# wittyseok/multimodal-organ-segmentation

Hardware: AMD Instinct MI355X
Metric: 96^3 2-modality patches/sec/node (train step) (higher is better)
Workload: dtype bf16; 1 GPU; DualEncoder fusion=cross_attention (mean, dual_encoder.py:193-195) 96^3, modalities CT+PET, 6 classes, DiceCE, AdamW, per-GPU batch 2; model=dual_encoder, global_batch=2, parallelism=dp1, kernels=hip, tag=c3

## Files before the change

include/mmseg_hip.h:

```cpp
#ifndef MMSEG_HIP_H
#define MMSEG_HIP_H

#include <stddef.h>
#include <stdint.h>

#ifdef __cplusplus
extern "C" {
#endif

const char* mmseg_last_error(void);
const char* mmseg_last_kernel(void);
int mmseg_abi_version(void);
int mmseg_timing_begin(void);
int mmseg_timing_end(void);
long long mmseg_timing_count(void);
int mmseg_timing_get(long long i, float* ms, const char** name);


int mmseg_pack_weight(const float* w, void* dst, int mode, int Co, int Ci, int Cip, int KG, int KGp, int Cpad,
                      int dtype, void* stream);

int mmseg_pack3_desc_bytes(void);
int mmseg_pack_conv3_batched(const void* descs, int n, int nblocks, int dtype, void* stream);
int mmseg_pack_desc_bytes(void);
// ... 58 lines not shown
                        const float* wdq, const float* bias, void* out, int ldo, int M, int Ncols, int Cpad, int KG,
                        int cpg_shift, int D, int H, int W, void* stream);
int mmseg_conv3_wgrad_norm_ok(long long V, int Co, int Cip, int Ci, int cpg_shift, int D, int H, int W, int lddy,
                              int ldx, int dtype);
int mmseg_conv3_wgrad_norm(const void* dy, int lddy, const void* x, int ldx, const float* nmean, const float* nrstd,
                           float* grad, float* bias_grad, int Co, int Cip, int Ci, int cpg_shift, long long V, int D,
                           int H, int W, float* ws, long long ws_floats, int accumulate, int dtype, void* stream);
int mmseg_conv_gemm_group(const void* a, int lda, const void* wpacked, const float* bias, void* out, int ldo,
                          float* splitk_ws, int mode, int M, int Ncols, int Cpad, int KG, int cpg_shift, int D, int H,
                          int W, int ksplit, int cin_real, int groups, long long w_gstride, int b_gstride, int dtype,
                          void* stream);
int mmseg_conv3_group_ok(int M, int Ncols, int Cpad, int KG, int cpg_shift, int D, int H, int W, int lda, int ldo,
                         int dtype);
int mmseg_conv3_wgrad_group_ok(long long V, int Co, int Cip, int Ci, int cpg_shift, int D, int H, int W, int lddy,
                               int ldx, int dtype);
int mmseg_conv3_group_splits(int M, int Ncols, int Cpad, int KG, int cpg_shift, int D, int H, int W, int lda, int ldo,
                             int dtype);
long long mmseg_conv3_wgrad_group_ws_floats(long long V, int Co, int Cip, int Ci, int cpg_shift, int D, int H, int W,
                                            int lddy, int ldx, int groups, int dtype);
int mmseg_conv3_wgrad_group(const void* dy, int lddy, const void* x, int ldx, float* grad, float* bias_grad, int Co,
                            int Cip, int Ci, int cpg_shift, long long V, int D, int H, int W, float* ws,
                            long long ws_floats, int accumulate, int groups, long long grad_gstride,
                            int bias_gstride, int phase, int dtype, void* stream);
int mmseg_wgrad_reduce_flush(void* stream);
int mmseg_wgrad_reduce_defer(const float* part, float* grad, const float* bias_part, float* bias_grad, int Ca,
                             int Ncols, int ksplit, int cpad, int creal, int ntap, int accumulate, void* stream);
int mmseg_wgrad_reduce_pending(void);
int mmseg_wgrad_reduce_discard(void* stream);
int mmseg_conv3_wgrad_ex(const void* dy, int lddy, const void* x, int ldx, const float* nmean, const float* nrstd,
                         float* grad, float* bias_grad, int Co, int Cip, int Ci, int cpg_shift, long long V, int D,
                         int H, int W, float* ws, long long ws_floats, int accumulate, int phase, int dtype,
                         void* stream);
int mmseg_colsum(const void* dy, int ld, int C, long long V, float* part, int nblk, float* out, int accumulate,
                 int dtype, void* stream);
int mmseg_colsum_reduce(const float* part, int nblk, int C, float* out, int accumulate, void* stream);

long long mmseg_instnorm_ws_floats(int N, long long V, int C);
int mmseg_instnorm_stats(const void* x, int ldx, int N, long long V, int C, float eps, float* mean, int mean_ld,
                         float* rstd, float* ws, int dtype, void* stream);
int mmseg_instnorm_relu_fwd(const void* x, int ldx, void* y, int ldy, int N, long long V, int C, const float* mean,
                            const float* rstd, int dtype, void* stream);
int mmseg_instnorm_relu_bwd_group(const void* x, int ldx, const float* mean, const float* rstd, const void* p1,
                                  int ld1, float scale1, int p1_nmod, const void* pool_dy, int pool_ld,
                                  const uint8_t* pool_idx, void* dx, int lddx, int N, int D, int H, int W, int C,
                                  float* ws, int dtype, void* stream);
int mmseg_instnorm_relu_bwd(const void* x, int ldx, const float* mean, const float* rstd, const void* p1, int ld1,
                            float scale1, const float* alpha1, int alpha_stride, const float* beta, int beta_stride,
                            const void* pool_dy, int pool_ld, const uint8_t* pool_idx, void* dx, int lddx, int N,
                            int D, int H, int W, int C, float* ws, int dtype, void* stream);
int mmseg_instnorm_act_bwd(const void* x, int ldx, const float* mean, const float* rstd, const void* g, int ldg,
                           void* dx, int lddx, int N, int D, int H, int W, int C, int Cw, int act, float slope,
                           const float* part, int nchunk, float* ws, int dtype, void* stream);
int mmseg_instnorm_part_chunks(long long V, int C);
int mmseg_lrelu_bwd_in_part(const void* y, int ldy, const void* dy, int lddy, void* g, int ldg, float slope,
                            const void* xa, int lda, const float* ma, const float* ra, float* pa, const void* xb,
                            int ldb, const float* mb, const float* rb, float* pb, int N, long long V, int C, int Cw,
                            int dtype, void* stream);
int mmseg_instnorm_fwd(const void* x, int ldx, void* y, int ldy, int N, long long V, int C, float eps, float* mean,
                       int mean_ld, float* rstd, int relu, float* ws, int dtype, void* stream);
int mmseg_instnorm_apply(const void* x, int ldx, void* y, int ldy, int N, long long V, int C, const float* mean,
                         const float* rstd, int relu, int dtype, void* stream);
int mmseg_instnorm_bwd(const void* x, int ldx, const float* mean, const float* rstd, const void* p1, int ld1,
                       float scale1, const float* alpha1, int alpha_stride, const float* beta, int beta_stride,
                       const void* pool_dy, int pool_ld, const uint8_t* pool_idx, void* dx, int lddx, int N, int D,
                       int H, int W, int C, int relu, float* ws, int dtype, void* stream);
int mmseg_instnorm_bwd_part(const void* x, int ldx, const float* mean, const float* rstd, const void* p1, int ld1,
                            float scale1, const float* alpha1, int alpha_stride, const float* beta, int beta_stride,
                            const void* pool_dy, int pool_ld, const uint8_t* pool_idx, void* dx, int lddx, int N,
                            int D, int H, int W, int C, int relu, const float* part, int nchunk, float* ws,
                            int dtype, void* stream);
int mmseg_instnorm_bwd_coef(const void* x, int ldx, const float* mean, const float* rstd, const void* p1, int ld1,
                            int N, int D, int H, int W, int C, int relu, const float* part, int nchunk,
                            float* coef, float* ws, int dtype, void* stream);
int mmseg_maxpool2_fwd(const void* x, int ldx, void* y, int ldy, uint8_t* idx, int N, int D, int H, int W, int C,
                       int dtype, void* stream);
int mmseg_maxpool2_norm_fwd(const void* x, int ldx, const float* mean, const float* rstd, void* y, int ldy,
                            uint8_t* idx, int N, int D, int H, int W, int C, int dtype, void* stream);

int mmseg_fuse_fwd(const void* const* srcs, const int* lds, int M, float wconst, const float* wts, void* out, int ldo,
                   int N, long long V, int C, int dtype, void* stream);
int mmseg_fuse_norm_fwd(const void* const* srcs, const int* lds, const float* const* means, const float* const* rstds,
                        int M, float wconst, const float* wts, void* out, int ldo, int N, long long V, int C,
                        int dtype, void* stream);
int mmseg_attn_gate_fwd(const float* pooled, const float* W1, const float* b1, const float* W2, const float* b2,
                        float* hbuf, float* wts, int N, int MC, int Hd, int M, void* stream);
int mmseg_attn_gate_bwd(const void* const* srcs, const int* lds, int M, const void* dfused, int ldd, int N, long long V,
                        int C, const float* pooled, const float* W1, const float* W2, const float* hbuf,
                        const float* wts, float* beta, float* gW1, float* gb1, float* gW2, float* gb2, int Hd,
                        float* ws, int accumulate, int dtype, void* stream);

int mmseg_bgemm_nt(const void* a, long long sa_outer, long long sa_inner, int lda, const void* b, long long sb_outer,
                   long long sb_inner, int ldb, void* c, long long sc_outer, long long sc_inner, int ldc,
                   const float* bias, int batch, int inner, int M, int N, int K, float alpha, int accumulate,
                   int c_dtype, int dtype, void* stream);
int mmseg_transpose(const void* src, long long s_outer, long long s_inner, int lds, int src_dtype, void* dst,
                    long long d_outer, long long d_inner, int ldd, int dst_dtype, int batch, int inner, int rows,
                    int cols, void* stream);
int mmseg_softmax_rows(const float* S, int lds, void* P, int ldp, long long rows, int N, int dtype, void* stream);
int mmseg_softmax_bwd_rows(const void* P, int ldp, const float* dP, int lddp, void* dS, int ldds, long long rows,
                           int N, int dtype, void* stream);

int mmseg_relpos_bias(const float* table, const int* index, int heads, int N, float* bias, void* stream);
int mmseg_softmax_bias_rows(const float* S, int lds, const float* bias, const float* mask, int nw, int heads, void* P,
                            int ldp, long long rows, int N, int dtype, void* stream);
int mmseg_relpos_table_grad(const void* dS, int ldn, int B, int heads, int N, float* dB, const int* offs,
                            const int* pairs, int T, float* gtable, int accumulate, int dtype, void* stream);

long long mmseg_winattn_lse_floats(int B, int heads);
int mmseg_winattn_fwd(const void* qkv, int B, int N, int C, int heads, const float* table, int T, int w0, int w1,
                      int w2, const uint8_t* region, int nw, float scale, void* O, float* lse, void* stream);
int mmseg_winattn_bwd(const void* qkv, const void* O, const void* dO, const float* lse, int B, int N, int C, int heads,
                      const float* table, int T, int w0, int w1, int w2, const uint8_t* region, int nw, float scale,
                      void* dqkv, void* dS, int ldn, void* stream);
int mmseg_winattn_sum_groups(int B, int N, int heads);
int mmseg_winattn_bwd_sum(const void* qkv, const void* O, const void* dO, const float* lse, int B, int N, int C,
                          int heads, const float* table, int T, int w0, int w1, int w2, const uint8_t* region, int nw,
                          float scale, void* dqkv, float* dsum, int ldn, void* stream);

int mmseg_layernorm_fwd(const void* x, int ldx, void* y, int ldy, long long rows, int C, const float* gamma,
                        const float* beta, float eps, float* mean, float* rstd, int dtype, void* stream);
long long mmseg_layernorm_bwd_ws_floats(long long rows, int C);
int mmseg_layernorm_bwd(const void* x, int ldx, const void* dy, int lddy, void* dx, int lddx, long long rows, int C,
                        const float* gamma, const float* mean, const float* rstd, int add_dx, float* dgamma,
                        float* dbeta, int accumulate, float* ws, int dtype, void* stream);
int mmseg_gelu_fwd(const void* h, void* y, long long n, int dtype, void* stream);
int mmseg_gelu_bwd(const void* h, const void* dy, void* dh, long long n, int dtype, void* stream);
int mmseg_add(const void* a, const void* b, void* out, long long n, int dtype, void* stream);
int mmseg_dropout(const void* x, void* y, long long rows, int C, long long V, int ncdhw, float p, long long seed,
                  int dtype, void* stream);
int mmseg_window_partition(const void* src, int ldx, int B, int D, int H, int W, int C, int w0, int w1, int w2,
                           int s0, int s1, int s2, int Dp, int Hp, int Wp, void* dst, int dtype, void* stream);
int mmseg_window_reverse(const void* win, int B, int D, int H, int W, int C, int w0, int w1, int w2, int s0, int s1,
                         int s2, int Dp, int Hp, int Wp, const void* add_src, int ld_add, void* dst, int ld_dst,
                         int dtype, void* stream);
int mmseg_merge_gather(const void* x, int ldx, int B, int D, int H, int W, int C, void* out, int dtype, void* stream);
int mmseg_merge_scatter(const void* dout, int B, int D, int H, int W, int C, void* dx, int lddx, int dtype,
                        void* stream);
int mmseg_patchify(const float* x, int B, int Cin, int D, int H, int W, int Kp, void* out, int dtype, void* stream);
int mmseg_res_apply(const void* a, int lda, const float* ma, const float* ra, const void* b, int ldb, const float* mb,
                    const float* rb, void* y, int ldy, int N, long long V, int C, int Cw, float slope, int dtype,
                    void* stream);
int mmseg_lrelu_bwd(const void* y, int ldy, const void* dy, int lddy, void* g, int ldg, long long rows, int C, int Cw,
                    float slope, int dtype, void* stream);

long long mmseg_normalize_ws_bytes(void);
int mmseg_modality_normalize(float* x, long long V, int kind, double lo, double hi, void* ws, void* stream);
int mmseg_resize_linear(const float* src, int C, int D, int H, int W, float* dst, int d, int h, int w, void* stream);
int mmseg_resize_nearest(const void* src, int label_bytes, int C, int D, int H, int W, void* dst, int d, int h, int w,
                         void* stream);
int mmseg_phantom(int S, int ncls, const double* geo, int M, const float* class_mean, const float* noise_sd,
                  const int* abs_noise, const unsigned long long* keys, void* label, int label_bytes, float* image,
                  void* stream);
int mmseg_augment(const float* src, int C, int D, int H, int W, const void* label, int label_bytes, int flip_mask,
                  int rot_k, const float* scale, const float* shift, int noise, double noise_mean, float noise_sd,
                  const unsigned long long* noise_key, float* dst, void* label_dst, void* stream);

int mmseg_window_gather(const float* vol, int N, int C, int D, int H, int W, const int* win, int nw, int r0, int r1,
                        int r2, float* out, void* stream);
int mmseg_window_accum(const float* logits, int N, int C, int D, int H, int W, int n, int z0, int y0, int x0, int r0,
                       int r1, int r2, float* out, void* stream);
int mmseg_window_norm(float* out, int N, int C, int D, int H, int W, const float* cz, const float* cy, const float* cx,
                      void* stream);

int mmseg_pack_input(const float* x, int Ctot, int c0, int cnt, int N, long long V, void* out, int dtype,
                     void* stream);
int mmseg_pack_input_compact(const float* x, int Ctot, int c0, int cnt, int N, long long V, void* out, int dtype,
// ... 70 lines not shown
```

multimodal-organ-segmentation_amd/csrc/norm_pool.hip:

```cpp
#include "mmseg_common.h"

#include <algorithm>

#include <stdlib.h>
#include <type_traits>

namespace {

constexpr int UNR = 4;

template <typename T>
__global__ void in_stats_partial(const T* __restrict__ x, int ld, int V, int C, int vpc, float* __restrict__ part) {
  const int n = blockIdx.y, chunk = blockIdx.x, nchunk = gridDim.x;
  const int C8 = C >> 3;
  const int lanes_v = 256 / C8;
  const int tid = threadIdx.x;
  const int cg = tid % C8, vl = tid / C8;
  const T* xn = x + (long long)n * V * ld + cg * 8;
  float mu[8], m2[8];
#pragma unroll
  for (int j = 0; j < 8; ++j) {
    mu[j] = 0.f;
    m2[j] = 0.f;
  }
// ... 1026 lines not shown
  int M;
  float wconst;
  const float* wts;
  const float* mean[4];
  const float* rstd[4];
};

template <typename T, bool NORM = false>
__global__ void fuse_fwd(FuseSrc s, T* __restrict__ out, int ldo, long long V, int N, int C) {
  const int C8 = C >> 3;
  const int total = N * (int)V * C8;
  for (int i = blockIdx.x * blockDim.x + threadIdx.x; i < total; i += gridDim.x * blockDim.x) {
    const int cg = i % C8;
    const long long nv = i / C8;
    const int n = (int)(nv / (int)V);
    float acc[8];
#pragma unroll
    for (int j = 0; j < 8; ++j) acc[j] = 0.f;
    for (int m = 0; m < s.M; ++m) {
      V8<T> a;
      a.load(reinterpret_cast<const T*>(s.p[m]) + nv * s.ld[m] + cg * 8);
      if constexpr (NORM) {
        float mu[8], rs[8];
        load8f(s.mean[m] + n * C + cg * 8, mu);
        load8f(s.rstd[m] + n * C + cg * 8, rs);
#pragma unroll
        for (int j = 0; j < 8; ++j) {
          const float h = (a.get(j) - mu[j]) * rs[j];
          a.set(j, h > 0.f ? h : 0.f);
        }
      }
      const float w = s.wts ? s.wts[n * s.M + m] : 1.f;
#pragma unroll
      for (int j = 0; j < 8; ++j) acc[j] = s.wts ? fmaf(a.get(j), w, acc[j]) : acc[j] + a.get(j);
    }
    V8<T> o;
#pragma unroll
    for (int j = 0; j < 8; ++j) o.set(j, s.wts ? acc[j] : acc[j] * s.wconst);
    o.store(out + nv * ldo + cg * 8);
  }
}

template <typename T, int MM>
__global__ void fuse_norm_fwd_m(FuseSrc s, T* __restrict__ out, int ldo, long long V, int N, int C) {
  const int C8 = C >> 3;
  const int total = N * (int)V * C8;
  const int stride = gridDim.x * blockDim.x;
  int i = blockIdx.x * blockDim.x + threadIdx.x;
  const int cg = i % C8;
  int cur_n = -1;
  float mu[MM][8], rs[MM][8];
  for (; i < total; i += stride) {
    const long long nv = i / C8;
    const int n = (int)(nv / (int)V);
    V8<T> a[MM];
#pragma unroll
    for (int m = 0; m < MM; ++m) a[m].load(reinterpret_cast<const T*>(s.p[m]) + nv * s.ld[m] + cg * 8);
    if (n != cur_n) {
#pragma unroll
      for (int m = 0; m < MM; ++m) {
        load8f(s.mean[m] + n * C + cg * 8, mu[m]);
        load8f(s.rstd[m] + n * C + cg * 8, rs[m]);
      }
      cur_n = n;
    }
    float acc[8];
#pragma unroll
    for (int j = 0; j < 8; ++j) acc[j] = 0.f;
#pragma unroll
    for (int m = 0; m < MM; ++m) {
#pragma unroll
      for (int j = 0; j < 8; ++j) {
        const float h = (a[m].get(j) - mu[m][j]) * rs[m][j];
        a[m].set(j, h > 0.f ? h : 0.f);
      }
      const float w = s.wts ? s.wts[n * s.M + m] : 1.f;
#pragma unroll
      for (int j = 0; j < 8; ++j) acc[j] = s.wts ? fmaf(a[m].get(j), w, acc[j]) : acc[j] + a[m].get(j);
    }
    V8<T> o;
#pragma unroll
    for (int j = 0; j < 8; ++j) o.set(j, s.wts ? acc[j] : acc[j] * s.wconst);
    o.store(out + nv * ldo + cg * 8);
  }
}

template <typename T>
__global__ void fuse_dot_partial(FuseSrc s, const T* __restrict__ dfused, int ldd, long long V, int C, long long vpc,
                                 float* __restrict__ part) {
  const int n = blockIdx.y, chunk = blockIdx.x, nchunk = gridDim.x;
  const int C8 = C >> 3;
  const int tid = threadIdx.x;
  float acc[4] = {0.f, 0.f, 0.f, 0.f};
  const long long v0 = (long long)chunk * vpc;
  long long v1 = v0 + vpc;
  if (v1 > V) v1 = V;
  const long long e0 = v0 * C8, e1 = v1 * C8;
  for (long long e = e0 + tid; e < e1; e += 256) {
    const long long v = e / C8;
    const int cg = (int)(e - v * C8);
    const long long nv = (long long)n * V + v;
    V8<T> d;
    d.load(dfused + nv * ldd + cg * 8);
    for (int m = 0; m < s.M; ++m) {
      V8<T> a;
      a.load(reinterpret_cast<const T*>(s.p[m]) + nv * s.ld[m] + cg * 8);
      float t = 0.f;
#pragma unroll
      for (int j = 0; j < 8; ++j) t = fmaf(a.get(j), d.get(j), t);
      acc[m] += t;
    }
  }
  __shared__ float red[4][4];
  const int lane = tid & 63, wave = tid >> 6;
  for (int m = 0; m < s.M; ++m) {
    float w = wave_sum(acc[m]);
    if (lane == 0) red[m][wave] = w;
  }
  __syncthreads();
  if (tid < s.M) part[((long long)n * nchunk + chunk) * 4 + tid] = red[tid][0] + red[tid][1] + red[tid][2] + red[tid][3];
}

__global__ void attn_gate_fwd(const float* __restrict__ pooled, const float* __restrict__ W1,
                              const float* __restrict__ b1, const float* __restrict__ W2, const float* __restrict__ b2,
                              float* __restrict__ hbuf, float* __restrict__ wts, int MC, int Hd, int M) {
  const int n = blockIdx.x;
  extern __shared__ float sh[];
  float* h = sh;
  for (int k = threadIdx.x; k < Hd; k += blockDim.x) {
    float a = 0.f;
    for (int i = 0; i < MC; ++i) a = fmaf(W1[(long long)k * MC + i], pooled[(long long)n * MC + i], a);
    a += b1[k];
    a = a > 0.f ? a : 0.f;
    h[k] = a;
    hbuf[(long long)n * Hd + k] = a;
  }
  __syncthreads();
  if (threadIdx.x == 0) {
    float lg[4];
    float mx = -INFINITY;
    for (int m = 0; m < M; ++m) {
      float a = 0.f;
      for (int k = 0; k < Hd; ++k) a = fmaf(W2[m * Hd + k], h[k], a);
      lg[m] = a + b2[m];
      mx = fmaxf(mx, lg[m]);
    }
    float se = 0.f;
    for (int m = 0; m < M; ++m) {
      lg[m] = expf(lg[m] - mx);
      se += lg[m];
    }
    for (int m = 0; m < M; ++m) wts[n * M + m] = lg[m] / se;
  }
}

__global__ void attn_gate_bwd(const float* __restrict__ dot_part, int nchunk, const float* __restrict__ pooled,
                              const float* __restrict__ W1, const float* __restrict__ W2,
                              const float* __restrict__ hbuf, const float* __restrict__ wts, float* __restrict__ beta,
                              float* __restrict__ gW1, float* __restrict__ gb1, float* __restrict__ gW2,
                              float* __restrict__ gb2, int N, int MC, int Hd, int M, long long V, int accumulate) {
  extern __shared__ float sh[];
  float* dlog = sh;
  float* dh = sh + N * M;
  const int tid = threadIdx.x;
  if (tid < N * M) {
    const int n = tid / M, m = tid % M;
// ... 399 lines not shown
int mmseg_maxpool2_fwd(const void* x, int ldx, void* y, int ldy, uint8_t* idx, int N, int D, int H, int W, int C,
                       int dtype, void* stream) {
  MMSEG_REQUIRE(C % 8 == 0 && ((D | H | W) & 1) == 0, "maxpool2: C%%8==0 and even dims required");
  MMSEG_REQUIRE((long long)N * (D / 2) * (H / 2) * (W / 2) * (C / 8) <= kGridStrideMax, "maxpool2: too many items");
  hipStream_t s = (hipStream_t)stream;
  const int grid = grid_for((long long)N * (D / 2) * (H / 2) * (W / 2) * (C / 8));
  if (dtype == MMSEG_BF16)
    MMSEG_LAUNCH(maxpool2_fwd<bf16_t>, dim3(grid), dim3(256), 0, s, (const bf16_t*)x, ldx, (bf16_t*)y, ldy, idx,
                       N, D, H, W, C, (const float*)nullptr, (const float*)nullptr);
  else
    MMSEG_LAUNCH(maxpool2_fwd<float>, dim3(grid), dim3(256), 0, s, (const float*)x, ldx, (float*)y, ldy, idx, N,
                       D, H, W, C, (const float*)nullptr, (const float*)nullptr);
  return mmseg::check_launch("maxpool2_fwd");
}

int mmseg_maxpool2_norm_fwd(const void* x, int ldx, const float* mean, const float* rstd, void* y, int ldy,
                            uint8_t* idx, int N, int D, int H, int W, int C, int dtype, void* stream) {
  MMSEG_REQUIRE(C % 8 == 0 && ((D | H | W) & 1) == 0, "maxpool2: C%%8==0 and even dims required");
  MMSEG_REQUIRE((long long)N * (D / 2) * (H / 2) * (W / 2) * (C / 8) <= kGridStrideMax, "maxpool2: too many items");
  hipStream_t s = (hipStream_t)stream;
  const int grid = grid_for((long long)N * (D / 2) * (H / 2) * (W / 2) * (C / 8));
  if (dtype == MMSEG_BF16)
    MMSEG_LAUNCH((maxpool2_fwd<bf16_t, true>), dim3(grid), dim3(256), 0, s, (const bf16_t*)x, ldx, (bf16_t*)y,
                       ldy, idx, N, D, H, W, C, mean, rstd);
  else
    MMSEG_LAUNCH((maxpool2_fwd<float, true>), dim3(grid), dim3(256), 0, s, (const float*)x, ldx, (float*)y, ldy,
                       idx, N, D, H, W, C, mean, rstd);
  return mmseg::check_launch("maxpool2_norm_fwd");
}

int mmseg_fuse_norm_fwd(const void* const* srcs, const int* lds, const float* const* means, const float* const* rstds,
                        int M, float wconst, const float* wts, void* out, int ldo, int N, long long V, int C,
                        int dtype, void* stream) {
  MMSEG_REQUIRE(M >= 1 && M <= 4 && C % 8 == 0, "fuse: 1 <= M <= 4 and C%%8==0");
  MMSEG_REQUIRE((long long)N * V * (C / 8) <= kGridStrideMax, "fuse: too many items");
  FuseSrc s{};
  for (int m = 0; m < M; ++m) {
    s.p[m] = srcs[m];
    s.ld[m] = lds[m];
    s.mean[m] = means[m];
    s.rstd[m] = rstds[m];
  }
  s.M = M;
  s.wconst = wconst;
  s.wts = wts;
  hipStream_t st = (hipStream_t)stream;
  const int grid = grid_for((long long)N * V * (C / 8));
  const bool cm = M >= 2 && ((long long)grid * 256) % (C / 8) == 0;
  auto run = [&](auto tag) {
    using T = decltype(tag);
    if (cm && M == 2)
      MMSEG_LAUNCH((fuse_norm_fwd_m<T, 2>), dim3(grid), dim3(256), 0, st, s, (T*)out, ldo, V, N, C);
    else if (cm && M == 3)
      MMSEG_LAUNCH((fuse_norm_fwd_m<T, 3>), dim3(grid), dim3(256), 0, st, s, (T*)out, ldo, V, N, C);
    else
      MMSEG_LAUNCH((fuse_fwd<T, true>), dim3(grid), dim3(256), 0, st, s, (T*)out, ldo, V, N, C);
  };
  if (dtype == MMSEG_BF16) run(bf16_t{});
  else run(float{});
  return mmseg::check_launch("fuse_norm_fwd");
}

int mmseg_fuse_fwd(const void* const* srcs, const int* lds, int M, float wconst, const float* wts, void* out, int ldo,
                   int N, long long V, int C, int dtype, void* stream) {
  MMSEG_REQUIRE(M >= 1 && M <= 4 && C % 8 == 0, "fuse: 1 <= M <= 4 and C%%8==0");
  MMSEG_REQUIRE((long long)N * V * (C / 8) <= kGridStrideMax, "fuse: too many items");
  FuseSrc s{};
  for (int m = 0; m < M; ++m) {
    s.p[m] = srcs[m];
    s.ld[m] = lds[m];
  }
  s.M = M;
  s.wconst = wconst;
  s.wts = wts;
  hipStream_t st = (hipStream_t)stream;
  const int grid = grid_for((long long)N * V * (C / 8));
  if (dtype == MMSEG_BF16)
    MMSEG_LAUNCH(fuse_fwd<bf16_t>, dim3(grid), dim3(256), 0, st, s, (bf16_t*)out, ldo, V, N, C);
  else
    MMSEG_LAUNCH(fuse_fwd<float>, dim3(grid), dim3(256), 0, st, s, (float*)out, ldo, V, N, C);
  return mmseg::check_launch("fuse_fwd");
}

int mmseg_attn_gate_fwd(const float* pooled, const float* W1, const float* b1, const float* W2, const float* b2,
                        float* hbuf, float* wts, int N, int MC, int Hd, int M, void* stream) {
  MMSEG_REQUIRE(M <= 4, "attn gate: M <= 4");
  MMSEG_LAUNCH(attn_gate_fwd, dim3(N), dim3(256), Hd * sizeof(float), (hipStream_t)stream, pooled, W1, b1, W2,
                     b2, hbuf, wts, MC, Hd, M);
  return mmseg::check_launch("attn_gate_fwd");
}

int mmseg_attn_gate_bwd(const void* const* srcs, const int* lds, int M, const void* dfused, int ldd, int N, long long V,
                        int C, const float* pooled, const float* W1, const float* W2, const float* hbuf,
                        const float* wts, float* beta, float* gW1, float* gb1, float* gW2, float* gb2, int Hd,
                        float* ws, int accumulate, int dtype, void* stream) {
  MMSEG_REQUIRE(M <= 4 && C % 8 == 0, "attn gate bwd: M <= 4");
  FuseSrc s{};
  for (int m = 0; m < M; ++m) {
    s.p[m] = srcs[m];
    s.ld[m] = lds[m];
  }
  s.M = M;
  long long want = 256 * 64;
  long long nch = (V * (C / 8) + want - 1) / want;
  if (nch > 256) nch = 256;
  long long vpc = (V + nch - 1) / nch;
  nch = (V + vpc - 1) / vpc;
  hipStream_t st = (hipStream_t)stream;
  if (dtype == MMSEG_BF16)
    MMSEG_LAUNCH(fuse_dot_partial<bf16_t>, dim3((int)nch, N), dim3(256), 0, st, s, (const bf16_t*)dfused, ldd, V,
                       C, vpc, ws);
  else
    MMSEG_LAUNCH(fuse_dot_partial<float>, dim3((int)nch, N), dim3(256), 0, st, s, (const float*)dfused, ldd, V, C,
                       vpc, ws);
  if (mmseg::check_launch("fuse_dot_partial")) return 1;
  const int MC = M * C;
  const size_t shm = (size_t)(N * M + N * Hd) * sizeof(float);
  MMSEG_LAUNCH(attn_gate_bwd, dim3(1), dim3(256), shm, st, ws, (int)nch, pooled, W1, W2, hbuf, wts, beta, gW1,
                     gb1, gW2, gb2, N, MC, Hd, M, V, accumulate);
  return mmseg::check_launch("attn_gate_bwd");
}

}
```

multimodal-organ-segmentation_amd/engine/programs.py:

```python
from __future__ import annotations

import contextlib
import ctypes
import os
from typing import Dict, List, Optional, Tuple

import torch
import torch.nn as nn

from .._lib import ptr
from .layers import Block, ConvT2, DySpec, GroupBlock, Head, Packer, Point, act_group_view
from .runtime import Act, FlatParams, Runtime


SMALL_IN_V = 4096


def _check_dims(D, H, W, levels):
    f = 1 << (levels - 1)
    if D % f or H % f or W % f:
        raise ValueError(
            f"spatial dims {D}x{H}x{W} must be divisible by {f} (the reference's size-mismatch "
            "interpolate branch, unet.py:108-109, is not on the engine path)")


class _Decoder:

    def __init__(self, rt: Runtime, up_blocks: nn.ModuleList, out_conv: nn.Conv3d, dropout: float,
                 flat: FlatParams, features: List[int]):
        self.rt, self.F = rt, features
        self.ups = [ConvT2(rt, d.up, flat) for d in up_blocks]
        self.blocks = [Block(rt, d.conv, flat) for d in up_blocks]
        self.head = Head(rt, out_conv, flat)
        self.p = dropout

    def descs(self):
        d = []
        for u in self.ups:
            d += u.descs()
        for b in self.blocks:
            d += b.descs()
        return d

    def setup(self, N, dims):
        rt, F = self.rt, self.F
        self.cat = [rt.act(N, *dims[l], 2 * F[l]) for l in range(len(F) - 1)]
        self.dout = [rt.act(N, *dims[l], F[l]) for l in range(len(F) - 1)]
        self.dsplit = []
        for l in range(len(F) - 1):
            c = self.cat[l]
            half = c.N * c.V * F[l]
            self.dsplit.append((Act(c.buf, 0, F[l], F[l], c.N, c.D, c.H, c.W),
                                Act(c.buf, half, F[l], F[l], c.N, c.D, c.H, c.W)))
        self.split_bwd = False

    def skip_slot(self, l: int) -> Act:
        return self.cat[l].slot(self.F[l], self.F[l])

    def dskip(self, l: int) -> Act:
        return self.dsplit[l][1] if self.split_bwd else self.skip_slot(l)

    def fwd(self, bottom: Act, training: bool, loss=None):
        h = bottom
        nl = len(self.F) - 1
        self.defer_head = loss is not None and os.environ.get("MMSEG_DEFER_HEAD_NORM", "1") != "0"
        for j in range(nl):
            l = nl - 1 - j
            self.ups[j].fwd(h, self.cat[l].slot(0, self.F[l]))
            self.blocks[j].defer_out = self.defer_head and j == nl - 1
            self.blocks[j].fwd(self.cat[l], self.dout[l])
            h = self.dout[l]
        dscale = None
        if training and self.p > 0:
            keep = torch.empty(h.N, h.C, device=self.rt.device).bernoulli_(1.0 - self.p)
            dscale = keep / (1.0 - self.p)
        if loss is not None:
            labels, spec, cw = loss
            if self.defer_head:
                x2, mu, rs = self.blocks[nl - 1].out_stats()
                return self.head.fwd_loss(x2, labels, spec, cw, dscale, norm=(mu, rs))
            return self.head.fwd_loss(h, labels, spec, cw, dscale)
        logits = torch.empty(h.N, self.head.C, h.D, h.H, h.W, dtype=torch.float32, device=self.rt.device)
        self.head.fwd(h, logits, dscale)
        return logits

    def bwd(self, bottom: Act, dlogits: Optional[torch.Tensor], accumulate: bool,
            gout: Optional[torch.Tensor] = None) -> Act:
        nl = len(self.F) - 1
        self.split_bwd = True
        dh = self.dout[0]
        hpart = None
        if gout is not None:
            hx = self.blocks[nl - 1].out_stats()[0] if self.defer_head else self.dout[0]
            nch = self.head.in_chunks(hx)
# ... 185 lines not shown
        self._setup_outnorm(N)
        if self.fusion == "attention":
            self.pooled_mean = [torch.empty(N, M * F[l], dtype=torch.float32, device=rt.device) for l in range(self.L)]
            self.gate_h = [torch.empty(N, M * F[l] // 4, dtype=torch.float32, device=rt.device) for l in range(self.L)]
            self.gate_w = [torch.empty(N, M, dtype=torch.float32, device=rt.device) for l in range(self.L)]
            self.gate_beta = [torch.empty(N, M * F[l], dtype=torch.float32, device=rt.device) for l in range(self.L)]

    def _setup_groups(self, N: int):
        rt, F, M, dims = self.rt, self.F, self.M, self.dims
        self.l0 = self.L
        self.pooled_g, self.dpooled_g, self.y_g, self.idx_g, self.rep = {}, {}, {}, {}, {}
        if not self.gblocks or self.multistream or os.environ.get("MMSEG_GROUP_SMALL", "1") == "0":
            return
        for l in range(self.L - 1, 0, -1):
            gb = self.gblocks[l]
            gb.setup(N, *dims[l])
            xin = self.pooled_c[l]
            if not gb.ok(xin):
                break
            self.pooled_g[l] = xin
            self.dpooled_g[l] = self.dpooled_c[l]
            self.y_g[l] = rt.act(M * N, *dims[l], F[l])
            self.idx_g[l] = self.idx_c[l]
            for mm in range(M):
                self.y[mm][l] = act_group_view(self.y_g[l], mm, N)
            self.l0 = l

    def _setup_outnorm(self, N: int):
        rt, F, M, dims = self.rt, self.F, self.M, self.dims
        self.x2c, self.statsc = {}, {}
        self.group_outnorm = (M > 1 and self.fusion in ("mean", "add") and not self.multistream
                              and os.environ.get("MMSEG_GROUP_SMALL", "1") != "0")
        if not self.group_outnorm:
            return
        for l in range(min(self.l0, self.L)):
            C = F[l]
            x2c = rt.act(M * N, *dims[l], C)
            stc = torch.empty(4, M * N * C, dtype=torch.float32, device=rt.device)
            for m in range(M):
                b = self.encs[m][l]
                b.setup(N, *dims[l])
                b.x2 = act_group_view(x2c, m, N)
                b.stats = stc[:, m * N * C:(m + 1) * N * C]
            self.x2c[l], self.statsc[l] = x2c, stc

    def fused_out(self, l: int) -> Act:
        return self.dec.skip_slot(l) if l < self.L - 1 else self.bottom

    def dfused(self, l: int) -> Act:
        return self.dec.dskip(l) if l < self.L - 1 else self.bottom

    def _fuse_fwd(self, l: int):
        L, s, code = self.rt.lib, self.rt.stream, self.rt.code
        out = self.fused_out(l)
        ys = [self.y[m][l] for m in range(self.M)]
        N, V, C = out.N, out.V, out.C
        if self.fusion == "concat":
            self.proj[l].fwd(self.ycat[l], out)
            return
        srcs = _ptr_array([y.ptr for y in ys])
        lds = _int_array([y.ld for y in ys])
        if self.fusion == "attention":
            g = self.gates[l]
            for m, y in enumerate(ys):
                ws = self.rt.ws(L.mmseg_instnorm_ws_floats(N, V, C))
                L.mmseg_instnorm_stats(y.ptr, y.ld, N, V, C, 0.0, self.pooled_mean[l].data_ptr() + m * C * 4,
                                       self.M * C, None, ptr(ws), code, s)
            lin1, lin2 = g.attention[2], g.attention[4]
            L.mmseg_attn_gate_fwd(ptr(self.pooled_mean[l]), ptr(lin1.weight), ptr(lin1.bias), ptr(lin2.weight),
                                  ptr(lin2.bias), ptr(self.gate_h[l]), ptr(self.gate_w[l]), N, self.M * C,
                                  lin1.weight.shape[0], self.M, s)
            L.mmseg_fuse_fwd(srcs, lds, self.M, 1.0, ptr(self.gate_w[l]), out.ptr, out.ld, N, V, C, code, s)
        else:
            wconst = 1.0 if self.fusion == "add" else 1.0 / self.M
            blks = [self.encs[m][l] for m in range(self.M)]
            if blks[0].defer_out:
                st = [b.out_stats() for b in blks]
                L.mmseg_fuse_norm_fwd(_ptr_array([t[0].ptr for t in st]), _int_array([t[0].ld for t in st]),
                                      _ptr_array([t[1].data_ptr() for t in st]), _ptr_array([t[2].data_ptr() for t in st]),
                                      self.M, wconst, None, out.ptr, out.ld, N, V, C, code, s)
            else:
                L.mmseg_fuse_fwd(srcs, lds, self.M, wconst, None, out.ptr, out.ld, N, V, C, code, s)

    def materialize_features(self):
        for m in range(self.M):
            for l in range(self.L):
                if self.encs[m][l].defer_out:
                    self.encs[m][l].materialize_out(self.y[m][l])

    def _streams(self):
        main = torch.cuda.current_stream(self.rt.device)
        if not self.multistream:
            return [main] * self.M
        if getattr(self, "_side", None) is None:
            self._side = [torch.cuda.Stream(self.rt.device) for _ in range(self.M - 1)]
        return [main] + self._side

    @property
    def multistream(self) -> bool:
        return self.M > 1 and os.environ.get("MMSEG_MODALITY_STREAMS", "0") != "0"

    def _on(self, streams, m):
        if streams[m] is streams[0]:
            return contextlib.nullcontext()
        streams[m].wait_stream(streams[0])
        return torch.cuda.stream(streams[m])

    @property
    def stream_level(self) -> int:
        return 2

    def _group_fwd_levels(self):
        L, code, s = self.rt.lib, self.rt.code, self.rt.stream
        for l in range(self.l0, self.L):
            if l > self.l0:
                prev = self.y_g[l - 1]
                L.mmseg_maxpool2_fwd(prev.ptr, prev.ld, self.pooled_g[l].ptr, self.pooled_g[l].ld,
                                     ptr(self.idx_g[l]), prev.N, *self.dims[l - 1], prev.C, code, s)
            self.gblocks[l].fwd(self.pooled_g[l], self.y_g[l])

    def _enc_fwd_levels(self, m: int, x: torch.Tensor, lo: int, hi: int, group_from: Optional[int] = None):
        L, code, s = self.rt.lib, self.rt.code, self.rt.stream
        N, Cx, D, H, W = x.shape
        blocks = self.encs[m]
        for l in range(lo, hi):
            if l == 0:
                self.xin_v[m] = _pack_input(self.rt, blocks[0], x, m, 1, self.xin[m])
                blocks[0].fwd(self.xin_v[m], self.y[m][0])
                continue
            prev = self.y[m][l - 1]
            pb = blocks[l - 1]
            if pb.defer_out:
                x2, mu, rs = pb.out_stats()
                L.mmseg_maxpool2_norm_fwd(x2.ptr, x2.ld, ptr(mu), ptr(rs), self.pooled[m][l].ptr, self.pooled[m][l].ld,
                                          ptr(self.idx[m][l]), N, *self.dims[l - 1], prev.C, code, s)
            else:
                L.mmseg_maxpool2_fwd(prev.ptr, prev.ld, self.pooled[m][l].ptr, self.pooled[m][l].ld,
                                     ptr(self.idx[m][l]), N, *self.dims[l - 1], prev.C, code, s)
            if l == group_from:
                continue
            blocks[l].fwd(self.pooled[m][l], self.y[m][l])

    def forward(self, x: torch.Tensor, training: bool, loss=None) -> torch.Tensor:
        N, Cx, D, H, W = x.shape
        if Cx != self.M:
            raise ValueError(f"DualEncoder expects {self.M} modalities, got {Cx} channels")
        self.setup(N, D, H, W)
        self.pack()
        defer = self.fusion in ("mean", "add") and os.environ.get("MMSEG_DEFER_ENC_NORM", "1") != "0"
        for m in range(self.M):
            for l in range(self.L):
                d = self.dims[l]
                self.encs[m][l].defer_out = defer and d[0] * d[1] * d[2] > SMALL_IN_V
        streams = self._streams()
        split = min(max(self.stream_level, 0), self.L)
        if self.l0 < self.L:
            for m in range(self.M):
                self._enc_fwd_levels(m, x, 0, self.l0 + 1, group_from=self.l0)
            self._group_fwd_levels()
        else:
            for m in range(self.M):
                self._enc_fwd_levels(m, x, 0, split)
            for m in range(self.M):
                with self._on(streams, m):
                    self._enc_fwd_levels(m, x, split, self.L)
        for m in range(1, self.M):
            if streams[m] is not streams[0]:
                streams[0].wait_stream(streams[m])
        for l in range(self.L):
            self._fuse_fwd(l)
        return self.dec.fwd(self.bottom, training, loss)

    def loss_ok(self) -> bool:
        return self.dec.head.loss_ok(self.dec.dout[0])

    def backward(self, dlogits: Optional[torch.Tensor], accumulate: bool, gout: Optional[torch.Tensor] = None):
        L, s, code = self.rt.lib, self.rt.stream, self.rt.code
        self.dec.bwd(self.bottom, dlogits, accumulate, gout)
        M = self.M
        if self.fusion in ("mean", "add"):
            self._encoders_bwd_streams(accumulate)
            return
        for l in range(self.L - 1, -1, -1):
            dfused = self.dfused(l)
            N, V, C = dfused.N, dfused.V, dfused.C
            base: List[DySpec] = []
            if self.fusion == "concat":
                self.proj[l].bwd(self.ycat[l], dfused, self.ycat[l], accumulate)
                base = [DySpec(p1=self.y[m][l]) for m in range(M)]
            elif self.fusion == "attention":
                g = self.gates[l]
                lin1, lin2 = g.attention[2], g.attention[4]
                ys = [self.y[m][l] for m in range(M)]
                ws = self.rt.ws(256 * 4 * N)
                fl = self.flat
                L.mmseg_attn_gate_bwd(_ptr_array([y.ptr for y in ys]), _int_array([y.ld for y in ys]), M,
                                      dfused.ptr, dfused.ld, N, V, C, ptr(self.pooled_mean[l]), ptr(lin1.weight),
                                      ptr(lin2.weight), ptr(self.gate_h[l]), ptr(self.gate_w[l]),
                                      ptr(self.gate_beta[l]), ptr(fl.grad(lin1.weight)), ptr(fl.grad(lin1.bias)),
                                      ptr(fl.grad(lin2.weight)), ptr(fl.grad(lin2.bias)), lin1.weight.shape[0],
                                      ptr(ws), int(accumulate), code, s)
                fl.mark(lin1.weight, lin1.bias, lin2.weight, lin2.bias)
                base = [DySpec(p1=dfused, alpha=self.gate_w[l], alpha_off=m, alpha_stride=M,
                               beta=self.gate_beta[l], beta_off=m * C, beta_stride=M * C) for m in range(M)]
            else:
                sc = 1.0 if self.fusion == "add" else 1.0 / M
                base = [DySpec(p1=dfused, scale1=sc) for _ in range(M)]
            for m in range(M):
                dy = base[m]
                if l < self.L - 1:
                    dy.pool_dy = self.dpooled[m][l + 1]
                    dy.pool_idx = self.idx[m][l + 1]
                blk = self.encs[m][l]
                if l > 0:
                    blk.bwd(self.pooled[m][l], dy, self.dpooled[m][l], accumulate)
                else:
                    blk.bwd(self.xin_v[m], dy, None, accumulate)


    def _encoders_bwd_streams(self, accumulate: bool):
        M = self.M
        sc = 1.0 if self.fusion == "add" else 1.0 / M
        streams = self._streams()
        split = min(max(self.stream_level, 0), self.L)

        def levels(m, hi, lo):
            for l in range(hi - 1, lo - 1, -1):
                dy = DySpec(p1=self.dfused(l), scale1=sc)
                if l < self.L - 1:
                    dy.pool_dy = self.dpooled[m][l + 1]
                    dy.pool_idx = self.idx[m][l + 1]
                blk = self.encs[m][l]
                if l > 0:
                    blk.bwd(self.pooled[m][l], dy, self.dpooled[m][l], accumulate)
                else:
                    blk.bwd(self.xin_v[m], dy, None, accumulate)
# ... 58 lines not shown
```

Baseline: 354.5 patches/s.

## Fuse encoder-level fusion with max-pool downsampling in one forward kernel

Adds a kernel that reads each modality's encoder output once per level, applies the deferred instance-norm plus ReLU, writes the mean/add fused feature, and also produces each modality's 2x max-pooled output and argmax indices. The forward path is reordered to run level by level, interleaving encoder blocks with this fused fuse+pool step, so the separate maxpool and fuse passes no longer each re-read the full-resolution activations. It changes the forward schedule and bypasses the grouped-encoder and stream paths. It also risks subtle differences in pooling semantics, since pooling now reads the in-kernel normalized values.

```diff
diff --git a/include/mmseg_hip.h b/include/mmseg_hip.h
--- a/include/mmseg_hip.h
+++ b/include/mmseg_hip.h
@@ -164,6 +164,9 @@
 int mmseg_fuse_norm_fwd(const void* const* srcs, const int* lds, const float* const* means, const float* const* rstds,
                         int M, float wconst, const float* wts, void* out, int ldo, int N, long long V, int C,
                         int dtype, void* stream);
+int mmseg_fuse_pool_fwd(const void* const* srcs, const int* lds, const float* const* means, const float* const* rstds,
+                        int M, float wconst, void* out, int ldo, void* const* ys, const int* ldys,
+                        uint8_t* const* idxs, int N, int D, int H, int W, int C, int dtype, void* stream);
 int mmseg_attn_gate_fwd(const float* pooled, const float* W1, const float* b1, const float* W2, const float* b2,
                         float* hbuf, float* wts, int N, int MC, int Hd, int M, void* stream);
 int mmseg_attn_gate_bwd(const void* const* srcs, const int* lds, int M, const void* dfused, int ldd, int N, long long V,
diff --git a/multimodal-organ-segmentation_amd/csrc/norm_pool.hip b/multimodal-organ-segmentation_amd/csrc/norm_pool.hip
--- a/multimodal-organ-segmentation_amd/csrc/norm_pool.hip
+++ b/multimodal-organ-segmentation_amd/csrc/norm_pool.hip
@@ -1132,6 +1132,101 @@
 #pragma unroll
     for (int j = 0; j < 8; ++j) o.set(j, s.wts ? acc[j] : acc[j] * s.wconst);
     o.store(out + nv * ldo + cg * 8);
+  }
+}
+
+struct FusePoolSrc {
+  const void* p[3];
+  int ld[3];
+  const float* mean[3];
+  const float* rstd[3];
+  void* y[3];
+  int ldy[3];
+  uint8_t* idx[3];
+  float wconst;
+};
+
+template <typename T, int MM, bool NORM>
+__global__ __launch_bounds__(256) void fuse_pool_fwd_m(FusePoolSrc s, T* __restrict__ out, int ldo, int N, int D,
+                                                       int H, int W, int C) {
+  const int C8 = C >> 3;
+  const int Do = D >> 1, Ho = H >> 1, Wo = W >> 1;
+  const int total = N * Do * Ho * Wo * C8;
+  const int i = blockIdx.x * blockDim.x + threadIdx.x;
+  if (i >= total) return;
+  const int cg = i % C8;
+  int q = i / C8;
+  const int xo = q % Wo;
+  q /= Wo;
+  const int yo = q % Ho;
+  q /= Ho;
+  const int zo = q % Do;
+  const int n = q / Do;
+  const long long in0 = ((long long)(n * D + 2 * zo) * H + 2 * yo) * (long long)W + 2 * xo;
+  const long long vo = ((long long)(n * Do + zo) * Ho + yo) * Wo + xo;
+  constexpr int TB = sizeof(T) == 2 ? 8 : (MM == 2 ? 4 : 2);
+  float mu[MM][8], rs[MM][8];
+  if constexpr (NORM) {
+#pragma unroll
+    for (int m = 0; m < MM; ++m) {
+      load8f(s.mean[m] + n * C + cg * 8, mu[m]);
+      load8f(s.rstd[m] + n * C + cg * 8, rs[m]);
+    }
+  }
+  float best[MM][8];
+  uint8_t bi[MM][8];
+#pragma unroll
+  for (int t0 = 0; t0 < 8; t0 += TB) {
+    V8<T> a[TB][MM];
+#pragma unroll
+    for (int u = 0; u < TB; ++u) {
+      const int t = t0 + u;
+      const long long vin = in0 + ((long long)(t >> 2) * H + ((t >> 1) & 1)) * W + (t & 1);
+#pragma unroll
+      for (int m = 0; m < MM; ++m) a[u][m].load(reinterpret_cast<const T*>(s.p[m]) + vin * s.ld[m] + cg * 8);
+    }
+#pragma unroll
+    for (int u = 0; u < TB; ++u) {
+      const int t = t0 + u;
+      const long long vin = in0 + ((long long)(t >> 2) * H + ((t >> 1) & 1)) * W + (t & 1);
+      float acc[8];
+#pragma unroll
+      for (int j = 0; j < 8; ++j) acc[j] = 0.f;
+#pragma unroll
+      for (int m = 0; m < MM; ++m) {
+        if constexpr (NORM) {
+#pragma unroll
+          for (int j = 0; j < 8; ++j) {
+            const float h = (a[u][m].get(j) - mu[m][j]) * rs[m][j];
+            a[u][m].set(j, h > 0.f ? h : 0.f);
+          }
+        }
+#pragma unroll
+        for (int j = 0; j < 8; ++j) {
+          const float v = a[u][m].get(j);
+          acc[j] = acc[j] + v;
+          if (t == 0 || v > best[m][j] || v != v) {
+            best[m][j] = v;
+            bi[m][j] = (uint8_t)t;
+          }
+        }
+      }
+      V8<T> o;
+#pragma unroll
+      for (int j = 0; j < 8; ++j) o.set(j, acc[j] * s.wconst);
+      o.store(out + vin * ldo + cg * 8);
+    }
+  }
+#pragma unroll
+  for (int m = 0; m < MM; ++m) {
+    V8<T> o;
+#pragma unroll
+    for (int j = 0; j < 8; ++j) o.set(j, best[m][j]);
+    o.store(reinterpret_cast<T*>(s.y[m]) + vo * s.ldy[m] + cg * 8);
+    uint2 packed;
+    packed.x = bi[m][0] | (bi[m][1] << 8) | (bi[m][2] << 16) | ((uint32_t)bi[m][3] << 24);
+    packed.y = bi[m][4] | (bi[m][5] << 8) | (bi[m][6] << 16) | ((uint32_t)bi[m][7] << 24);
+    *reinterpret_cast<uint2*>(s.idx[m] + vo * C + cg * 8) = packed;
   }
 }
 
@@ -1697,6 +1792,49 @@
   return mmseg::check_launch("fuse_fwd");
 }
 
+int mmseg_fuse_pool_fwd(const void* const* srcs, const int* lds, const float* const* means, const float* const* rstds,
+                        int M, float wconst, void* out, int ldo, void* const* ys, const int* ldys,
+                        uint8_t* const* idxs, int N, int D, int H, int W, int C, int dtype, void* stream) {
+  MMSEG_REQUIRE((M == 2 || M == 3) && C % 8 == 0 && C > 0, "fuse_pool: M in {2, 3} and C%%8==0 required");
+  MMSEG_REQUIRE(N > 0 && D > 0 && H > 0 && W > 0 && ((D | H | W) & 1) == 0, "fuse_pool: even dims required");
+  MMSEG_REQUIRE((means == nullptr) == (rstds == nullptr), "fuse_pool: means and rstds go together");
+  const long long total = (long long)N * (D / 2) * (H / 2) * (W / 2) * (C / 8);
+  MMSEG_REQUIRE(total <= kGridStrideMax && (long long)N * D < 2147483647LL, "fuse_pool: too many items");
+  FusePoolSrc s{};
+  for (int m = 0; m < M; ++m) {
+    MMSEG_REQUIRE(srcs[m] && ys[m] && idxs[m] && lds[m] >= C && ldys[m] >= C && lds[m] % 8 == 0 && ldys[m] % 8 == 0,
+                  "fuse_pool: source / pooled rows of at least C, multiples of 8");
+    s.p[m] = srcs[m];
+    s.ld[m] = lds[m];
+    if (means) {
+      MMSEG_REQUIRE(means[m] && rstds[m], "fuse_pool: statistics of every source");
+      s.mean[m] = means[m];
+      s.rstd[m] = rstds[m];
+    }
+    s.y[m] = ys[m];
+    s.ldy[m] = ldys[m];
+    s.idx[m] = idxs[m];
+  }
+  MMSEG_REQUIRE(out && ldo >= C && ldo % 8 == 0, "fuse_pool: output rows of at least C, a multiple of 8");
+  s.wconst = wconst;
+  hipStream_t st = (hipStream_t)stream;
+  const int grid = (int)((total + 255) / 256);
+  auto run = [&](auto tag) {
+    using T = decltype(tag);
+    if (M == 2 && means)
+      MMSEG_LAUNCH((fuse_pool_fwd_m<T, 2, true>), dim3(grid), dim3(256), 0, st, s, (T*)out, ldo, N, D, H, W, C);
+    else if (M == 2)
+      MMSEG_LAUNCH((fuse_pool_fwd_m<T, 2, false>), dim3(grid), dim3(256), 0, st, s, (T*)out, ldo, N, D, H, W, C);
+    else if (means)
+      MMSEG_LAUNCH((fuse_pool_fwd_m<T, 3, true>), dim3(grid), dim3(256), 0, st, s, (T*)out, ldo, N, D, H, W, C);
+    else
+      MMSEG_LAUNCH((fuse_pool_fwd_m<T, 3, false>), dim3(grid), dim3(256), 0, st, s, (T*)out, ldo, N, D, H, W, C);
+  };
+  if (dtype == MMSEG_BF16) run(bf16_t{});
+  else run(float{});
+  return mmseg::check_launch("fuse_pool_fwd");
+}
+
 int mmseg_attn_gate_fwd(const float* pooled, const float* W1, const float* b1, const float* W2, const float* b2,
                         float* hbuf, float* wts, int N, int MC, int Hd, int M, void* stream) {
   MMSEG_REQUIRE(M <= 4, "attn gate: M <= 4");
diff --git a/multimodal-organ-segmentation_amd/engine/programs.py b/multimodal-organ-segmentation_amd/engine/programs.py
--- a/multimodal-organ-segmentation_amd/engine/programs.py
+++ b/multimodal-organ-segmentation_amd/engine/programs.py
@@ -10,6 +10,7 @@
 
 from .._lib import ptr
 from .layers import Block, ConvT2, DySpec, GroupBlock, Head, Packer, Point, act_group_view
+from .profiler import TIMER
 from .runtime import Act, FlatParams, Runtime
 
 
@@ -361,6 +362,47 @@
             else:
                 L.mmseg_fuse_fwd(srcs, lds, self.M, wconst, None, out.ptr, out.ld, N, V, C, code, s)
 
+    def _fuse_pool_fwd(self, l: int):
+        L, s, code = self.rt.lib, self.rt.stream, self.rt.code
+        out = self.fused_out(l)
+        M = self.M
+        blks = [self.encs[m][l] for m in range(M)]
+        if l < self.l0 and blks[0].defer_out:
+            st = [b.out_stats() for b in blks]
+            srcs = [t[0] for t in st]
+            means = _ptr_array([t[1].data_ptr() for t in st])
+            rstds = _ptr_array([t[2].data_ptr() for t in st])
+        else:
+            srcs = [self.y[m][l] for m in range(M)]
+            means = rstds = None
+        pooled = [self.pooled[m][l + 1] for m in range(M)]
+        wconst = 1.0 if self.fusion == "add" else 1.0 / M
+        es = self.rt.dtype.itemsize
+        nvox = out.N * out.V
+        with TIMER.region("fuse_pool_fwd_m",
+                          nbytes=float(es * out.C * (M * nvox + nvox + M * nvox // 8) + M * out.C * nvox // 8)):
+            L.mmseg_fuse_pool_fwd(_ptr_array([a.ptr for a in srcs]), _int_array([a.ld for a in srcs]), means, rstds,
+                                  M, wconst, out.ptr, out.ld, _ptr_array([p.ptr for p in pooled]),
+                                  _int_array([p.ld for p in pooled]),
+                                  _ptr_array([ptr(self.idx[m][l + 1]) for m in range(M)]),
+                                  out.N, *self.dims[l], out.C, code, s)
+
+    def _fwd_fuse_pool(self, x: torch.Tensor):
+        for l in range(self.L):
+            if l >= self.l0:
+                self.gblocks[l].fwd(self.pooled_g[l], self.y_g[l])
+            else:
+                for m in range(self.M):
+                    if l == 0:
+                        self.xin_v[m] = _pack_input(self.rt, self.encs[m][0], x, m, 1, self.xin[m])
+                        self.encs[m][0].fwd(self.xin_v[m], self.y[m][0])
+                    else:
+                        self.encs[m][l].fwd(self.pooled[m][l], self.y[m][l])
+            if l < self.L - 1:
+                self._fuse_pool_fwd(l)
+            else:
+                self._fuse_fwd(l)
+
     def materialize_features(self):
         for m in range(self.M):
             for l in range(self.L):
@@ -431,6 +473,11 @@
             for l in range(self.L):
                 d = self.dims[l]
                 self.encs[m][l].defer_out = defer and d[0] * d[1] * d[2] > SMALL_IN_V
+        self.fuse_pool = (self.fusion in ("mean", "add") and self.M in (2, 3) and not self.multistream
+                          and os.environ.get("MMSEG_FUSE_POOL", "1") != "0")
+        if self.fuse_pool:
+            self._fwd_fuse_pool(x)
+            return self.dec.fwd(self.bottom, training, loss)
         streams = self._streams()
         split = min(max(self.stream_level, 0), self.L)
         if self.l0 < self.L:
```

Result: faster. 358.5 patches/s, median of 6 (+1.1%).
